# kakaobrain/rq-vae-transformer

Hardware: AMD Instinct MI355X
Metric: 256x256 images/sec, AR sampling + decode (RQ-Transformer huge, 8x8x4 codes) (higher is better)
Workload: dtype bf16

## Files before the change

rq-vae-transformer_amd/csrc/conv_halo.hip:

```cpp
#include <stdlib.h>
#include <type_traits>
#include "gemm.h"
#include "rq_common.h"
#include "vae_kernels.h"
#ifndef RQ_CONV_NT
#define RQ_CONV_NT 0
#endif
#ifndef RQ_CONVOUT_NT
#define RQ_CONVOUT_NT 0
#endif
static __device__ __forceinline__ rq_u128 ld128_act(const void* p) {
#if RQ_CONV_NT >= 2
    return ld128_nt(p);
#else
    return ld128(p);
#endif
}
static __device__ __forceinline__ void st128_act(void* p, rq_u128 v) {
#if RQ_CONV_NT >= 1
    st128_nt(p, v);
#else
    st128(p, v);
#endif
}

struct ConvHaloArgs {
    const bf16_t* x;
    const bf16_t* w;
    const float* bias;
    const float* gn;
    const bf16_t* resid;
    bf16_t* out;
    float* stats;
    int B, H, W, Cin, Cout;
};

#define RQ_LOG2E 1.4426950408889634f
static __device__ __forceinline__ float rq_silu_l2(float t) { return t * rq_fast_rcp(fmaf(rq_fast_exp2(-t), RQ_LOG2E, RQ_LOG2E)); }

static __device__ __forceinline__ void rq_stats_piece(const rq_u128& u, float (&sum)[4], float (&sq)[4]) {
    const uint32_t w[4] = {u.x, u.y, u.z, u.w};
#pragma unroll
    for (int e = 0; e < 4; ++e) {
        sum[e] = rq_dot2_bf16(w[e], RQ_ONE_X2, sum[e]);
        sq[e] = rq_dot2_bf16(w[e], w[e], sq[e]);
    }
}

constexpr int HT_H = 8, HT_W = 32;
constexpr int HP_W = HT_W + 2;
constexpr int H_BN = 128;
constexpr int HW_BYTES = H_BN * 128;
#ifndef RQ_HALO_WDMA
#define RQ_HALO_WDMA 1
#endif
#ifndef RQ_HALO_PMID
#define RQ_HALO_PMID 0
#endif
#ifndef RQ_HALO_RMID
#define RQ_HALO_RMID 1
#endif
#ifndef RQ_HALO_RES_F32
#define RQ_HALO_RES_F32 1
#endif
constexpr int H_WSLOTS = RQ_HALO_WDMA ? 4 : 3;
constexpr int H_SMEM_BYTES = 2 * (HT_H + 2) * HP_W * 128 + H_WSLOTS * HW_BYTES;
static __device__ __forceinline__ void halo_wait_dma(int nd, int no) {
#define RQ_HC(ND, K) case K: rq_wait_vmcnt_mixed<ND, K>(); break;
#define RQ_HW(ND) switch (no) { RQ_HC(ND, 0) RQ_HC(ND, 1) RQ_HC(ND, 2) RQ_HC(ND, 3) RQ_HC(ND, 4) RQ_HC(ND, 5) RQ_HC(ND, 6) RQ_HC(ND, 7) RQ_HC(ND, 8) \
    RQ_HC(ND, 9) RQ_HC(ND, 10) RQ_HC(ND, 11) RQ_HC(ND, 12) default: rq_wait_vmcnt_mixed<ND, 0>(); break; }
    if (nd >= 2) { RQ_HW(2) } else { RQ_HW(0) }
#undef RQ_HW
#undef RQ_HC
}

template <int PW = HP_W>
static __device__ __forceinline__ unsigned halo_lds_off(int hy, int hx, int c8) {
    return (unsigned)((hy * PW + hx) * 128 + ((c8 ^ ((hx >> 1) & 7)) << 4));
}

#ifdef RQ_CONV_TRACE
__device__ unsigned long long g_conv_trace[8 * 64];
#define RQ_CT(slot) do { if (blockIdx.x == RQ_CONV_TRACE && lane == 0 && (slot) < 64) g_conv_trace[wave * 64 + (slot)] = __builtin_readcyclecounter(); } while (0)
#else
#define RQ_CT(slot) do { } while (0)
#endif
template <int FUSE_GN, int UPS, int RES>
__global__ __launch_bounds__(512, 1) void conv3x3_halo_kernel(ConvHaloArgs p) {
    constexpr bool WDMA = RQ_HALO_WDMA != 0;
    constexpr int TH = HT_H, NTH = 512, RPW = 2, NJ = 2, W_IT = 2, TPX = TH * HT_W, W_SETS = 3, W_SLOTS = H_WSLOTS;
    static_assert(!(FUSE_GN && UPS), "the upsample conv has no Normalize in front of it");
    constexpr int PW = UPS ? HT_W / 2 + 2 : HP_W, PH = UPS ? TH / 2 + 2 : TH + 2;
    constexpr int HP_N = PW * PH;
    constexpr int HALO_BYTES = HP_N * 128;
    constexpr int H_IT = (HP_N * 8 + NTH - 1) / NTH;
    RQ_DYN_SMEM(smem);
    char* sH = (char*)smem;
    char* sW = sH + 2 * HALO_BYTES;
    const int tid = threadIdx.x, lane = tid & 63, wave = tid >> 6;
    const int wm = wave >> 1, wn = wave & 1;
#ifdef RQ_CONV_TRACE
    if (blockIdx.x == RQ_CONV_TRACE && lane == 0) g_conv_trace[wave * 64 + 58] = __builtin_amdgcn_s_memrealtime();
#endif

    const int tiles_x = p.W / HT_W, tiles_y = p.H / TH, NT = p.Cout / H_BN;
    const int n_mt = p.B * tiles_y * tiles_x;
    const int id = blockIdx.x, xcd = id & 7, slot = id >> 3;
    const int per = (n_mt + 7) >> 3;
    const int mtile = xcd * per + slot / NT;
    const int nt = slot - (slot / NT) * NT;
    if (slot >= per * NT || mtile >= n_mt) return;
    const int img = mtile / (tiles_y * tiles_x);
    const int trem = mtile - img * (tiles_y * tiles_x);
    const int ty0 = (trem / tiles_x) * TH, tx0 = (trem - (trem / tiles_x) * tiles_x) * HT_W;
    const int n0 = nt * H_BN;

    const char* gX = (const char*)p.x;
    const char* gWt = (const char*)p.w;
    const int w_row = tid >> 3, w_c8 = tid & 7;
    unsigned w_goff[W_IT];
#pragma unroll
    for (int i = 0; i < W_IT; ++i) w_goff[i] = (unsigned)(((long)(n0 + w_row + (NTH / 8) * i) * 9 * p.Cin + w_c8 * 8) * 2);
    auto load_w = [&](int c, int tap, rq_u128* rw) {
        const unsigned kb = (unsigned)(tap * p.Cin + c * 64) * 2u;
#pragma unroll
        for (int i = 0; i < W_IT; ++i) rw[i] = ld128(gWt + (w_goff[i] + kb));
    };
    rq_u128 rh[H_IT], rw[W_SETS][W_IT], r01[2][W_IT];
    unsigned w_voff[2];
#pragma unroll
    for (int i = 0; i < 2; ++i) {
        const int r = wave * 16 + i * 8 + (lane >> 3);
        w_voff[i] = (unsigned)(((long)(n0 + r) * 9 * p.Cin + ((lane & 7) ^ ((r >> 1) & 7)) * 8) * 2);
    }
    const rq_lds_t sW_dma = rq_lds_addr(sW) + (rq_lds_t)rq_uniform(wave) * 2048u;
    auto dma_w = [&](int c, int tap, unsigned woff) {
        if (tap >= 9) { tap -= 9; ++c; }
        rq_glds16_s2(sW_dma + woff, gWt + (unsigned)rq_uniform((tap * p.Cin + c * 64) * 2), w_voff[0], w_voff[1]);
    };
    if (WDMA) {
        dma_w(0, 0, 0u);
        dma_w(0, 1, (unsigned)HW_BYTES);
        dma_w(0, 2, 2u * HW_BYTES);
    } else {
        load_w(0, 0, r01[0]);
        load_w(0, 1, r01[1]);
        load_w(0, 2, rw[2]);
        load_w(0, 3, rw[0]);
        load_w(0, 4, rw[1]);
    }
    rq_sched_barrier();

    unsigned hd[H_IT];
    const int Hs = UPS ? p.H >> 1 : p.H, Ws = UPS ? p.W >> 1 : p.W;
    const unsigned x_img = (unsigned)((long)img * Hs * Ws * p.Cin * 2) + (unsigned)((tid & 7) * 16);
    const unsigned cin2 = (unsigned)p.Cin * 2u;
    const int hp0 = tid >> 3, hy0 = hp0 / PW, hx0 = hp0 - hy0 * PW;
    {
        int hy = hy0, hx = hx0;
#pragma unroll
        for (int it = 0; it < H_IT; ++it) {
            const int gy = (UPS ? ty0 >> 1 : ty0) + hy - 1, gx = (UPS ? tx0 >> 1 : tx0) + hx - 1;
            const int cy = gy < 0 ? 0 : (gy >= Hs ? Hs - 1 : gy), cx = gx < 0 ? 0 : (gx >= Ws ? Ws - 1 : gx);
            hd[it] = (unsigned)(cy * Ws + cx);
            rh[it] = ld128_act(gX + (x_img + hd[it] * cin2));
            hy += (NTH / 8) / PW; hx += (NTH / 8) % PW;
            if (hx >= PW) { hx -= PW; ++hy; }
        }
    }
    const float* gn = FUSE_GN ? p.gn + (long)img * p.Cin * 2 : nullptr;
    f32x4 gs[4];
    auto load_gs = [&](int c) {
        if (FUSE_GN) {
#pragma unroll
            for (int e = 0; e < 4; ++e) gs[e] = *(const f32x4*)(gn + (c * 64 + (tid & 7) * 8 + e * 2) * 2);
        }
    };
    auto scale_gs = [&]() {
        if (FUSE_GN) {
#pragma unroll
            for (int e = 0; e < 4; ++e) { rq_opaque_f4(gs[e]); gs[e] = gs[e] * RQ_LOG2E; }
        }
    };
    load_gs(0);
    rq_sched_barrier();
    {
        int hp = hp0, hy = hy0, hx = hx0;
        const int c8 = tid & 7;
#pragma unroll
        for (int it = 0; it < H_IT; ++it) {
            const bool in = hp < HP_N;
            const int gy = (UPS ? ty0 >> 1 : ty0) + hy - 1, gx = (UPS ? tx0 >> 1 : tx0) + hx - 1;
            const bool ok = in && gy >= 0 && gy < Hs && gx >= 0 && gx < Ws;
            const unsigned loff16 = in ? halo_lds_off<PW>(hy, hx, c8) >> 4 : 0u;
            hd[it] |= (loff16 << 16) | (ok ? 1u << 29 : 0u) | (in ? 1u << 30 : 0u);
            hp += NTH / 8; hy += (NTH / 8) / PW; hx += (NTH / 8) % PW;
            if (hx >= PW) { hx -= PW; ++hy; }
        }
    }
    auto h_in = [&](int it) { return (hd[it] >> 30) & 1u; };
    auto h_ok = [&](int it) { return (hd[it] >> 29) & 1u; };
    auto h_loff = [&](int it) { return ((hd[it] >> 16) & 0x1fffu) << 4; };
    auto h_goff = [&](int it) { return x_img + (hd[it] & 0xffffu) * cin2; };
    auto load_halo_piece = [&](int c, rq_u128* rh, int it) { rh[it] = ld128_act(gX + (h_goff(it) + (unsigned)c * 128u)); };

    unsigned w_loff[W_IT];
#pragma unroll
    for (int i = 0; i < W_IT; ++i) {
        const int r = w_row + (NTH / 8) * i;
        w_loff[i] = (unsigned)(r * 128 + ((w_c8 ^ ((r >> 1) & 7)) << 4));
    }
    auto halo_piece_value = [&](const rq_u128* rh, int it) -> rq_u128 {
        rq_u128 v = rh[it];
        if (FUSE_GN) {
            float f[8];
            rq_unpack2(v.x, f[0], f[1]);
            rq_unpack2(v.y, f[2], f[3]);
            rq_unpack2(v.z, f[4], f[5]);
            rq_unpack2(v.w, f[6], f[7]);
#pragma unroll
            for (int e = 0; e < 8; e += 2) {
                const f32x4 ss = gs[e >> 1];
                const float a = fmaf(f[e], ss[0], ss[1]), b = fmaf(f[e + 1], ss[2], ss[3]);
                f[e] = rq_silu_l2(a);
                f[e + 1] = rq_silu_l2(b);
            }
            v.x = pack_bf16x2(f[0], f[1]); v.y = pack_bf16x2(f[2], f[3]);
            v.z = pack_bf16x2(f[4], f[5]); v.w = pack_bf16x2(f[6], f[7]);
        }
        if (!h_ok(it)) v = zero128();
        return v;
    };
    auto halo_word = [&](rq_u128* rh, int it, int e) -> uint32_t& { return e == 0 ? rh[it].x : e == 1 ? rh[it].y : e == 2 ? rh[it].z : rh[it].w; };
    auto halo_piece_word = [&](rq_u128* rh, int it, int e) {
        uint32_t& w = halo_word(rh, it, e);
        if (FUSE_GN) {
            const f32x4 ss = gs[e];
            float wlo, whi;
            rq_unpack2(w, wlo, whi);
            const float a = fmaf(wlo, ss[0], ss[1]), b = fmaf(whi, ss[2], ss[3]);
            w = pack_bf16x2(rq_silu_l2(a), rq_silu_l2(b));
        }
        if (!h_ok(it)) w = 0u;
    };
    auto store_w = [&](int wslot, const rq_u128* rw) {
#pragma unroll
        for (int i = 0; i < W_IT; ++i) st128(sW + wslot * HW_BYTES + w_loff[i], rw[i]);
    };

    f32x16 acc[RPW][NJ];
#pragma unroll
    for (int j = 0; j < NJ; ++j)
#pragma unroll
        for (int q = 0; q < 4; ++q) {
            const f32x4 bv = *(const f32x4*)(p.bias + n0 + wn * (NJ * 32) + j * 32 + 8 * q + 4 * (lane >> 5));
#pragma unroll
            for (int i = 0; i < RPW; ++i)
#pragma unroll
                for (int e = 0; e < 4; ++e) acc[i][j][4 * q + e] = bv[e];
        }

    const int ftx = lane & 31, fk = lane >> 5;
    const unsigned rd_w0 = (unsigned)((wn * (NJ * 32) + ftx) * 128 + ((fk ^ ((ftx >> 1) & 7)) << 4));
    unsigned rd_h0[3];
#pragma unroll
    for (int kx = 0; kx < 3; ++kx)
        rd_h0[kx] = UPS ? halo_lds_off<PW>(wm * (RPW / 2), (ftx + kx + 1) >> 1, fk) : halo_lds_off<PW>(wm * RPW, ftx + kx, fk);

    auto load_frags = [&](int hbuf, unsigned woff, int ky, int kx, int ks, bf16x8* af, bf16x8* bfr) {
        const char* hb = sH + ((rd_h0[kx] + (unsigned)(hbuf * HALO_BYTES)) ^ (unsigned)(ks << 5));
        const char* wb = sW + ((rd_w0 ^ (unsigned)(ks << 5)) + woff);
#pragma unroll
        for (int i = 0; i < RPW; ++i) af[i] = as_bf16x8(ld128(hb + (UPS ? (i + ky + 1) >> 1 : i + ky) * (PW * 128)));
#pragma unroll
        for (int j = 0; j < NJ; ++j) bfr[j] = as_bf16x8(ld128(wb + j * (32 * 128)));
    };
#ifndef RQ_HALO_FDEPTH
#define RQ_HALO_FDEPTH 1
#endif
    constexpr int FD = RQ_HALO_FDEPTH, NSET = FD + 1;
    static_assert(FD >= 1 && FD <= 3 && 36 % NSET == 0, "fragment read-ahead of 1..3 k-steps");
    bf16x8 fa[NSET][RPW], fb[NSET][NJ];
    auto mfma_step = [&](int set) {
#pragma unroll
        for (int i = 0; i < RPW; ++i)
#pragma unroll
            for (int j = 0; j < NJ; ++j) acc[i][j] = rq_mfma_32x32x16_bf16(fb[set][j], fa[set][i], acc[i][j]);
    };

    const int NC = p.Cin / 64, last_c = NC - 1;
    auto load_unit = [&](int c, int tap, rq_u128* r) {
        if (tap >= 9) { tap -= 9; ++c; }
        if (c > last_c) return false;
        load_w(c, tap, r);
        return true;
    };
    {
        RQ_CT(0);
        scale_gs();
#pragma unroll
        for (int it = 0; it < H_IT; ++it)
            if (h_in(it)) st128(sH + h_loff(it), halo_piece_value(rh, it));
        if (WDMA) rq_wait_vmcnt_mixed<0, 0>();
// ... 537 lines not shown
                for (int k = 0; k < PPT; ++k) {
                    const int it = (tap - FIRST) * PPT + k;
                    if (ptap && it < H_IT) rh[it] = halo_piece_value(rh, it);
                }
                compute(hbuf, wbuf, ky, kx, rh, -1);
            }
            store_w(wbuf ^ 1, rw[(tap + 1) % W_SETS]);
#pragma unroll
            for (int k = 0; k < PPT; ++k) {
                const int it = (tap - FIRST) * PPT + k;
                if (!(ptap && it < H_IT)) continue;
                if (h_in(it)) st128(sH + (hbuf ^ 1) * PK_PSTRIDE + h_loff(it), rh[it]);
            }
            RQ_CTP(2 + (c * 9 + tap) * 2);
            rq_syncthreads();
            RQ_CTP(3 + (c * 9 + tap) * 2);
            wbuf ^= 1;
        }
        hbuf ^= 1;
    };

    for (;;) {
        rq_opaque(tid_o);
        static_assert(CPR == 16 && NTH / CPR == HT_W && R_IT == TH, "piece k = tile row k");
        if (SUB)
            io_off0 = (unsigned)((((long)cur.img * p.H + 2 * cur.ty0 + (cur.cls >> 1)) * p.W + 2 * (cur.tx0 + (tid_o >> 4)) + (cur.cls & 1)) * p.Cout + cur.n0 + (tid_o & 15) * 8) * 2u;
        else
            io_off0 = (unsigned)((((long)cur.img * p.H + cur.ty0) * p.W + cur.tx0 + (tid_o >> 4)) * p.Cout + cur.n0 + (tid_o & 15) * 8) * 2u;
        RQ_CTP(1);
        for (int c = 0; c + 1 < NC; ++c) run_chunk(c, std::false_type{});
        run_chunk(NC - 1, std::true_type{});

        char* sT = (char*)smem + PK_P0 + (hbuf == 0 ? PK_PATCH : 0);
        const int lane_o = tid_o & 63, wave_o = tid_o >> 6, wm_o = wave_o >> 1, wn_o = wave_o & 1;
        float* sred = (float*)(sT + PK_TILE);
        if (RES) {
#pragma unroll
            for (int k = 0; k < R_IT; ++k) st128(sT + ((tid_o >> 4) + HT_W * k) * PK_LDR + (tid_o & 15) * 16, rr[k]);
            rq_syncthreads();
        }
#pragma unroll
        for (int i = 0; i < RPW; ++i) {
            const int ty = wm_o * RPW + i, tx = lane_o & 31;
            const int ml = ty * HT_W + tx;
#pragma unroll
            for (int j = 0; j < 2; ++j) {
#pragma unroll
                for (int q = 0; q < 4; ++q) {
                    const int nl = wn_o * 64 + j * 32 + 8 * q + 4 * (lane_o >> 5);
                    float v[4];
#pragma unroll
                    for (int e = 0; e < 4; ++e) v[e] = acc[i][j][4 * q + e];
                    if (RES) {
                        const uint32_t* rp = (const uint32_t*)(sT + ml * PK_LDR + nl * 2);
                        const uint32_t r0 = rp[0], r1 = rp[1];
                        { float lo_, hi_; rq_unpack2(r0, lo_, hi_); v[0] += lo_; v[1] += hi_; }
                        { float lo_, hi_; rq_unpack2(r1, lo_, hi_); v[2] += lo_; v[3] += hi_; }
                    }
                    struct __attribute__((aligned(8))) u64 { uint32_t a, b; } w2;
                    w2.a = pack_bf16x2(v[0], v[1]);
                    w2.b = pack_bf16x2(v[2], v[3]);
                    *(u64*)(sT + ml * PK_LDR + nl * 2) = w2;
                }
            }
        }
        if (has_next) acc_from_bias(nxt.n0);
        rq_syncthreads();
        RQ_CTP(61);
        float gs_[4], gq_[4];
#pragma unroll
        for (int e = 0; e < 4; ++e) { gs_[e] = 0.f; gq_[e] = 0.f; }
#pragma unroll
        for (int k = 0; k < R_IT; ++k) {
            const rq_u128 u = ld128(sT + ((tid_o >> 4) + HT_W * k) * PK_LDR + (tid_o & 15) * 16);
            st128_act((char*)p.out + (io_off0 + (unsigned)k * io_step), u);
            if (p.stats) rq_stats_piece(u, gs_, gq_);
        }
        if (p.stats) {
            const int gsz = p.Cout / 32;
            float a0, q0, a1, q1;
            if (gsz == 4) {
                a0 = gs_[0] + gs_[1]; q0 = gq_[0] + gq_[1];
                a1 = gs_[2] + gs_[3]; q1 = gq_[2] + gq_[3];
            } else {
                a0 = (gs_[0] + gs_[1]) + (gs_[2] + gs_[3]);
                q0 = (gq_[0] + gq_[1]) + (gq_[2] + gq_[3]);
                a1 = 0.f; q1 = 0.f;
            }
            a0 += rq_shfl_xor(a0, 16); q0 += rq_shfl_xor(q0, 16); a1 += rq_shfl_xor(a1, 16); q1 += rq_shfl_xor(q1, 16);
            a0 += rq_shfl_xor(a0, 32); q0 += rq_shfl_xor(q0, 32); a1 += rq_shfl_xor(a1, 32); q1 += rq_shfl_xor(q1, 32);
            if (lane_o < 16) {
                float* o = sred + (wave_o * 16 + lane_o) * 4;
                o[0] = a0; o[1] = q0; o[2] = a1; o[3] = q1;
            }
            rq_syncthreads();
            if (wave_o == 0) {
                const int chunk = (lane_o >> 1) & 15, pair = lane_o & 1;
                float a = 0.f, q = 0.f;
#pragma unroll
                for (int w = 0; w < NTH / 64; ++w) { a += sred[(w * 16 + chunk) * 4 + pair * 2]; q += sred[(w * 16 + chunk) * 4 + pair * 2 + 1]; }
                if (gsz == 16) {
                    a += rq_shfl_xor(a, 2);
                    q += rq_shfl_xor(q, 2);
                }
                const bool writer = gsz == 4 ? true : (gsz == 8 ? pair == 0 : (pair == 0 && (chunk & 1) == 0));
                if (writer && lane_o < 32) {
                    const int g = (cur.n0 + chunk * 8 + pair * 4) / gsz;
                    const int tiles = tiles_x * tiles_y * NCLS;
                    float* o = p.stats + (((long)cur.img * tiles + cur.trem) * 32 + g) * 2;
                    o[0] = a;
                    o[1] = q;
                }
            }
        }
        RQ_CTP(63);
#ifdef RQ_CONV_TRACE
        ++trace_tile;
#endif
        if (!has_next) break;
        rq_use(rw[1][0].x, rw[1][1].x, rw[2][0].x, rw[2][1].x);
        if (SUB) rq_use(rw[W_SETS - 1][0].x, rw[W_SETS - 1][1].x, rw[W_SETS - 1][0].y, rw[W_SETS - 1][1].y);
        rq_use(acc[0][0][0], acc[RPW - 1][1][15]);
        slot += wpx;
        cur = nxt;
        wn_cur = wn_nxt;
        if (SUB) set_class(cur.cls);
        has_next = slot_ok(slot + wpx);
        if (has_next) { nxt = decode(slot + wpx); wn_nxt = (unsigned)nxt.n0 * w_per_n + (unsigned)nxt.cls * w_per_cls; }
    }
}

struct ConvOutArgs {
    const bf16_t* x;
    const float* w;
    const float* bias;
    const float* gn;
    float* y;
    int B, H, W, Cin, Cout;
};
constexpr int OT_H = 4, OP_N = (OT_H + 2) * HP_W;
constexpr int O_NTH = 256;
constexpr int O_PLANE = OP_N * 128;

template <int FUSE_GN>
__global__ __launch_bounds__(O_NTH) void conv_out_halo_kernel(ConvOutArgs p) {
    RQ_DYN_SMEM(smem);
    const int NC = p.Cin / 64;
    char* sH = (char*)smem;
    const int wrow = 9 * p.Cin * 2 + 32;
    char* sW = sH + NC * O_PLANE;
    const int tid = threadIdx.x, lane = tid & 63, wave = rq_uniform(tid >> 6);

    const int tiles_x = p.W / HT_W, tiles_y = p.H / OT_H, tiles_img = tiles_x * tiles_y;
    const int n_mt = p.B * tiles_img;
    const int id = blockIdx.x, xcd = id & 7, slot = id >> 3, S = (int)gridDim.x >> 3;
    const int per = (n_mt + 7) >> 3;
    const int x0 = xcd * per, x1 = x0 + per < n_mt ? x0 + per : n_mt;
    const int sub = (x1 - x0 + S - 1) / (S > 0 ? S : 1);
    const int t0 = x0 + slot * sub, t1 = t0 + sub < x1 ? t0 + sub : x1;
    if (x0 >= x1 || t0 >= t1) return;

    const int cpp_sh = p.Cin == 64 ? 3 : 4;
    const int CPP = 1 << cpp_sh;
    const int cq = tid & (CPP - 1);
    const int n_piece = OP_N << cpp_sh;
    constexpr int PIT = 13;
    unsigned hyx[PIT];
#pragma unroll
    for (int k = 0; k < PIT; ++k) {
        const int q = tid + O_NTH * k;
        const int hp = q >> cpp_sh;
        const int hy = hp / HP_W, hx = hp - hy * HP_W;
        hyx[k] = q < n_piece ? (unsigned)(hy << 8 | hx) : 0xffffu;
    }
    const char* gX = (const char*)p.x;
    struct Tile { int img, ty0, tx0; };
    auto decode = [&](int t) {
        Tile d;
        d.img = t / tiles_img;
        const int trem = t - d.img * tiles_img;
        d.ty0 = (trem / tiles_x) * OT_H;
        d.tx0 = (trem - (trem / tiles_x) * tiles_x) * HT_W;
        return d;
    };
    auto request = [&](const Tile& d, rq_u128* r, f32x4* gs) {
        if (FUSE_GN) {
            const float* gn = p.gn + ((long)d.img * p.Cin + cq * 8) * 2;
#pragma unroll
            for (int e = 0; e < 4; ++e) gs[e] = *(const f32x4*)(gn + e * 4) * RQ_LOG2E;
        }
#pragma unroll
        for (int k = 0; k < PIT; ++k) {
            if (hyx[k] == 0xffffu) continue;
            const int gy = d.ty0 + (int)(hyx[k] >> 8) - 1, gx = d.tx0 + (int)(hyx[k] & 255u) - 1;
            const int cy = gy < 0 ? 0 : (gy >= p.H ? p.H - 1 : gy), cx = gx < 0 ? 0 : (gx >= p.W ? p.W - 1 : gx);
#if RQ_CONVOUT_NT
            r[k] = ld128_nt(gX + ((((long)d.img * p.H + cy) * p.W + cx) * p.Cin + cq * 8) * 2);
#else
            r[k] = ld128(gX + ((((long)d.img * p.H + cy) * p.W + cx) * p.Cin + cq * 8) * 2);
#endif
        }
    };
    auto stage = [&](const Tile& d, const rq_u128* r, const f32x4* gs) {
#pragma unroll
        for (int k = 0; k < PIT; ++k) {
            if (hyx[k] == 0xffffu) continue;
            const int hy = (int)(hyx[k] >> 8), hx = (int)(hyx[k] & 255u);
            const int gy = d.ty0 + hy - 1, gx = d.tx0 + hx - 1;
            rq_u128 v = r[k];
            if (FUSE_GN) {
                float f[8];
                rq_unpack2(v.x, f[0], f[1]);
                rq_unpack2(v.y, f[2], f[3]);
                rq_unpack2(v.z, f[4], f[5]);
                rq_unpack2(v.w, f[6], f[7]);
#pragma unroll
                for (int e = 0; e < 8; e += 2) {
                    const f32x4 ss = gs[e >> 1];
                    const float a = fmaf(f[e], ss[0], ss[1]), b = fmaf(f[e + 1], ss[2], ss[3]);
                    f[e] = rq_silu_l2(a);
                    f[e + 1] = rq_silu_l2(b);
                }
                v.x = pack_bf16x2(f[0], f[1]); v.y = pack_bf16x2(f[2], f[3]);
                v.z = pack_bf16x2(f[4], f[5]); v.w = pack_bf16x2(f[6], f[7]);
            }
            if (gy < 0 || gy >= p.H || gx < 0 || gx >= p.W) v = zero128();
            st128(sH + (unsigned)((cq >> 3) * O_PLANE) + halo_lds_off(hy, hx, cq & 7), v);
        }
    };

    rq_u128 r[PIT];
    f32x4 gs[4];
    Tile cur = decode(t0);
    request(cur, r, gs);
    const int KT = 9 * p.Cin;
    const int n_w4 = p.Cout * (KT >> 2);
    constexpr int WIT = 5;
    {
        f32x4 wr[WIT];
#pragma unroll
        for (int k = 0; k < WIT; ++k) {
            const int i = tid + O_NTH * k;
            if (i < n_w4) wr[k] = *(const f32x4*)(p.w + (long)i * 4);
        }
        stage(cur, r, gs);
#pragma unroll
        for (int k = 0; k < WIT; ++k) {
            const int i = tid + O_NTH * k;
            if (i < n_w4) {
                const int row = i / (KT >> 2), k4 = (i - row * (KT >> 2)) * 4;
                *(uint64_t*)(sW + row * wrow + k4 * 2) = (uint64_t)pack_bf16x2(wr[k][0], wr[k][1]) | ((uint64_t)pack_bf16x2(wr[k][2], wr[k][3]) << 32);
            }
        }
        for (int i = n_w4 + tid; i < 8 * (KT >> 2); i += O_NTH) {
            const int row = i / (KT >> 2), k4 = (i - row * (KT >> 2)) * 4;
            *(uint64_t*)(sW + row * wrow + k4 * 2) = 0ull;
        }
    }

    const int ftx = lane & 31, fk = lane >> 5;
    const char* wl = sW + (ftx & 7) * wrow + fk * 16;
    float bias_r[4];
#pragma unroll
    for (int co = 0; co < 4; ++co) bias_r[co] = co < p.Cout ? p.bias[co] : 0.f;
    for (int t = t0; t < t1; ++t) {
        const bool more = t + 1 < t1;
        Tile nxt = cur;
        if (more) { nxt = decode(t + 1); request(nxt, r, gs); }
        rq_syncthreads();
        f32x16 acc;
#pragma unroll
        for (int q = 0; q < 16; ++q) acc[q] = 0.f;
        constexpr int OD = 4;
        for (int c = 0; c < NC; ++c) {
            bf16x8 af[OD + 1], wf[OD + 1];
            auto frag = [&](int s, bf16x8& a, bf16x8& w) {
                const int tap = s >> 2, ks = s & 3, ky = tap / 3, kx = tap - ky * 3;
                const unsigned ha = (unsigned)(c * O_PLANE) + halo_lds_off(wave + ky, ftx + kx, fk);
                a = as_bf16x8(ld128(sH + (ha ^ (unsigned)(ks << 5))));
                w = as_bf16x8(ld128(wl + (tap * p.Cin + c * 64) * 2 + ks * 32));
            };
#pragma unroll
            for (int s = 0; s < OD; ++s) frag(s, af[s], wf[s]);
#pragma unroll
            for (int s = 0; s < 36; ++s) {
                if (s + OD < 36) frag(s + OD, af[(s + OD) % (OD + 1)], wf[(s + OD) % (OD + 1)]);
                acc = rq_mfma_32x32x16_bf16(wf[s % (OD + 1)], af[s % (OD + 1)], acc);
                rq_sched_barrier();
            }
        }
        if (lane < 32) {
            const int oy = cur.ty0 + wave, ox = cur.tx0 + lane;
#pragma unroll
            for (int co = 0; co < 4; ++co)
                if (co < p.Cout) p.y[(((long)cur.img * p.Cout + co) * p.H + oy) * p.W + ox] = acc[co] + bias_r[co];
        }
        if (!more) break;
        rq_syncthreads();
        stage(nxt, r, gs);
        cur = nxt;
    }
}

bool rq_conv_out_halo_supported(int H, int W, int Cin, int Cout) {
    return H % OT_H == 0 && W % HT_W == 0 && (Cin == 64 || Cin == 128) && Cout >= 1 && Cout <= 4;
}

int rq_launch_conv_out_halo(const bf16_t* x, const float* w, const float* bias, const float* gn, float* y, int B, int H, int W,
                            int Cin, int Cout, hipStream_t s) {
    if (!rq_conv_out_halo_supported(H, W, Cin, Cout)) return rq_fail(RQAMD_ERR_UNSUPPORTED, "conv_out_halo: shape %dx%d %d->%d", H, W, Cin, Cout);
    ConvOutArgs a{};
    a.x = x; a.w = w; a.bias = bias; a.gn = gn; a.y = y; a.B = B; a.H = H; a.W = W; a.Cin = Cin; a.Cout = Cout;
    const size_t smem = (size_t)(Cin / 64) * O_PLANE + 8 * (size_t)(9 * Cin * 2 + 32);
    static RqDeviceOnce attr_once;
    if (attr_once.first()) {
        (void)hipFuncSetAttribute((const void*)conv_out_halo_kernel<0>, hipFuncAttributeMaxDynamicSharedMemorySize, 160 * 1024);
        (void)hipFuncSetAttribute((const void*)conv_out_halo_kernel<1>, hipFuncAttributeMaxDynamicSharedMemorySize, 160 * 1024);
    }
    const int n_mt = B * (H / OT_H) * (W / HT_W);
    int nblocks = 8 * ((n_mt + 7) / 8);
    int cus = 256;
    (void)hipDeviceGetAttribute(&cus, hipDeviceAttributeMultiprocessorCount, 0);
    if (nblocks > 2 * cus) nblocks = 2 * cus / 8 * 8;
    if (const char* e = getenv("RQAMD_CONV_OUT_WGS")) {
        const int v = atoi(e) / 8 * 8;
        if (v >= 8 && v < nblocks) nblocks = v;
    }
    if (gn) RQ_LAUNCH(conv_out_halo_kernel<1>, dim3(nblocks), dim3(O_NTH), smem, s, a);
    else RQ_LAUNCH(conv_out_halo_kernel<0>, dim3(nblocks), dim3(O_NTH), smem, s, a);
    return rq_check_launch("conv_out_halo_kernel");
}

struct ConvInArgs {
    const float* x;
    const float* w;
    const float* bias;
    bf16_t* y;
    float* stats;
    int B, H, W;
};
constexpr int CI_COUT = 128, CI_PATCH = 3 * (HT_H + 2) * HP_W;
constexpr int CI_WROW = 80;
constexpr int CI_STG = 32 * (CI_COUT * 2 + 16);

__global__ __launch_bounds__(256) void conv_in_mfma_kernel(ConvInArgs p) {
    RQ_DYN_SMEM(smem);
    float* sP = (float*)smem;
    int* sK = (int*)(smem + 4096);
    char* sWt = (char*)smem + 4096 + 128;
    char* sO = sWt + CI_COUT * CI_WROW;
    const int tid = threadIdx.x, lane = tid & 63, wave = rq_uniform(tid >> 6);
    const int tiles_x = p.W / HT_W, tiles_y = p.H / HT_H;
    const int tile = blockIdx.x;
    const int img = tile / (tiles_y * tiles_x), trem = tile - img * (tiles_y * tiles_x);
    const int ty0 = (trem / tiles_x) * HT_H, tx0 = (trem - (trem / tiles_x) * tiles_x) * HT_W;

    for (int i = tid; i < CI_PATCH + 4; i += 256) {
        float v = 0.f;
        if (i < CI_PATCH) {
            const int ci = i / ((HT_H + 2) * HP_W), r = i - ci * ((HT_H + 2) * HP_W);
            const int hy = r / HP_W, hx = r - hy * HP_W;
            const int gy = ty0 + hy - 1, gx = tx0 + hx - 1;
            if (gy >= 0 && gy < p.H && gx >= 0 && gx < p.W) v = p.x[(((long)img * 3 + ci) * p.H + gy) * p.W + gx];
        }
        sP[i] = v;
    }
    if (tid < 32) {
        const int k = tid, tap = k / 3, ci = k - tap * 3, ky = tap / 3, kx = tap - ky * 3;
        sK[k] = k < 27 ? ci * ((HT_H + 2) * HP_W) + ky * HP_W + kx : -1;
    }
    for (int i = tid; i < CI_COUT * 16; i += 256) {
        const int co = i >> 4, k2 = (i & 15) * 2;
        const float a = k2 < 27 ? p.w[k2 * CI_COUT + co] : 0.f, b = k2 + 1 < 27 ? p.w[(k2 + 1) * CI_COUT + co] : 0.f;
        *(uint32_t*)(sWt + co * CI_WROW + k2 * 2) = pack_bf16x2(a, b);
    }
    rq_syncthreads();

    const int px = lane & 31, g = lane >> 5;
    int koff[2][8];
#pragma unroll
    for (int ks = 0; ks < 2; ++ks)
#pragma unroll
        for (int e = 0; e < 8; ++e) koff[ks][e] = sK[ks * 16 + g * 8 + e];
    bf16x8 bfr[2][4];
#pragma unroll
    for (int ks = 0; ks < 2; ++ks)
#pragma unroll
        for (int j = 0; j < 4; ++j) bfr[ks][j] = as_bf16x8(ld128(sWt + (j * 32 + px) * CI_WROW + (ks * 16 + g * 8) * 2));
    char* stg = sO + wave * CI_STG;
    float gs_[4] = {0.f, 0.f, 0.f, 0.f}, gq_[4] = {0.f, 0.f, 0.f, 0.f};
#pragma unroll 1
    for (int i = 0; i < 2; ++i) {
        const int row = wave * 2 + i;
        f32x16 acc[4];
#pragma unroll
        for (int j = 0; j < 4; ++j)
#pragma unroll
            for (int r = 0; r < 16; ++r) acc[j][r] = 0.f;
#pragma unroll
        for (int ks = 0; ks < 2; ++ks) {
            float f[8];
#pragma unroll
            for (int e = 0; e < 8; ++e) f[e] = koff[ks][e] >= 0 ? sP[koff[ks][e] + row * HP_W + px] : 0.f;
            rq_u128 u;
            u.x = pack_bf16x2(f[0], f[1]); u.y = pack_bf16x2(f[2], f[3]);
            u.z = pack_bf16x2(f[4], f[5]); u.w = pack_bf16x2(f[6], f[7]);
            const bf16x8 af = as_bf16x8(u);
#pragma unroll
            for (int j = 0; j < 4; ++j) acc[j] = rq_mfma_32x32x16_bf16(bfr[ks][j], af, acc[j]);
        }
#pragma unroll
        for (int j = 0; j < 4; ++j)
#pragma unroll
            for (int q = 0; q < 4; ++q) {
                const int co = j * 32 + 8 * q + 4 * g;
                const f32x4 bv = *(const f32x4*)(p.bias + co);
                struct __attribute__((aligned(8))) u64 { uint32_t a, b; } w2;
                w2.a = pack_bf16x2(acc[j][4 * q] + bv[0], acc[j][4 * q + 1] + bv[1]);
                w2.b = pack_bf16x2(acc[j][4 * q + 2] + bv[2], acc[j][4 * q + 3] + bv[3]);
                *(u64*)(stg + px * (CI_COUT * 2 + 16) + co * 2) = w2;
            }
        rq_syncthreads();
        const long pix0 = ((long)img * p.H + ty0 + row) * p.W + tx0;
#pragma unroll
        for (int k = 0; k < 8; ++k) {
            const int c = lane + 64 * k, opx = c >> 4, part = c & 15;
            const rq_u128 u = ld128(stg + opx * (CI_COUT * 2 + 16) + part * 16);
            st128(p.y + (pix0 + opx) * CI_COUT + part * 8, u);
            if (p.stats) rq_stats_piece(u, gs_, gq_);
        }
        rq_syncthreads();
    }
    if (p.stats) {
        float a0 = gs_[0] + gs_[1], q0 = gq_[0] + gq_[1], a1 = gs_[2] + gs_[3], q1 = gq_[2] + gq_[3];
        a0 += rq_shfl_xor(a0, 16); q0 += rq_shfl_xor(q0, 16); a1 += rq_shfl_xor(a1, 16); q1 += rq_shfl_xor(q1, 16);
        a0 += rq_shfl_xor(a0, 32); q0 += rq_shfl_xor(q0, 32); a1 += rq_shfl_xor(a1, 32); q1 += rq_shfl_xor(q1, 32);
        float* sred = (float*)sO;
        if (lane < 16) {
            float* o = sred + (wave * 16 + lane) * 4;
            o[0] = a0; o[1] = q0; o[2] = a1; o[3] = q1;
        }
        rq_syncthreads();
        if (tid < 32) {
            const int chunk = tid >> 1, pair = tid & 1;
            float a = 0.f, q = 0.f;
#pragma unroll
            for (int w = 0; w < 4; ++w) { a += sred[(w * 16 + chunk) * 4 + pair * 2]; q += sred[(w * 16 + chunk) * 4 + pair * 2 + 1]; }
            float* o = p.stats + (((long)img * (tiles_y * tiles_x) + trem) * 32 + tid) * 2;
            o[0] = a;
            o[1] = q;
        }
    }
}

bool rq_conv_in_mfma_supported(int H, int W, int Cin, int Cout) {
    return Cin == 3 && Cout == CI_COUT && H % HT_H == 0 && W % HT_W == 0;
}

int rq_launch_conv_in_mfma(const float* x, const float* w, const float* bias, bf16_t* y, float* stats, int B, int H, int W, hipStream_t s) {
    ConvInArgs a{};
    a.x = x; a.w = w; a.bias = bias; a.y = y; a.stats = stats; a.B = B; a.H = H; a.W = W;
    const size_t smem = 4096 + 128 + (size_t)CI_COUT * CI_WROW + 4 * (size_t)CI_STG;
    static RqDeviceOnce attr_once;
    if (attr_once.first()) {
        (void)hipFuncSetAttribute((const void*)conv_in_mfma_kernel, hipFuncAttributeMaxDynamicSharedMemorySize, (int)smem);
    }
    RQ_LAUNCH(conv_in_mfma_kernel, dim3((unsigned)(B * (H / HT_H) * (W / HT_W))), dim3(256), smem, s, a);
    return rq_check_launch("conv_in_mfma_kernel");
}

__global__ __launch_bounds__(256) void gn_params_kernel(const float* part, const float* gamma, const float* beta, float* gn, int B, int HW,
                                                        int C, int nchunk, float eps) {
    __shared__ float sa[8][32], sq[8][32], smean[32], srstd[32];
    const int b = blockIdx.x, tid = threadIdx.x, g = tid & 31, sl = tid >> 5;
    float a = 0.f, q = 0.f;
    for (int c = sl; c < nchunk; c += 8) {
        const float* o = part + (((long)b * nchunk + c) * 32 + g) * 2;
        a += o[0];
        q += o[1];
    }
    sa[sl][g] = a;
    sq[sl][g] = q;
    rq_syncthreads();
    if (tid < 32) {
        float ta = 0.f, tq = 0.f;
#pragma unroll
        for (int k = 0; k < 8; ++k) { ta += sa[k][tid]; tq += sq[k][tid]; }
        const float n = (float)HW * (float)(C / 32);
        const float mean = ta / n;
        float var = tq / n - mean * mean;
        if (var < 0.f) var = 0.f;
        smean[tid] = mean;
        srstd[tid] = 1.0f / sqrtf(var + eps);
    }
    rq_syncthreads();
    const int cpg = C / 32;
    for (int ch = tid; ch < C; ch += 256) {
        const int gg = ch / cpg;
        const float sc = srstd[gg] * gamma[ch];
        gn[((long)b * C + ch) * 2] = sc;
        gn[((long)b * C + ch) * 2 + 1] = beta[ch] - smean[gg] * sc;
    }
}

__global__ void ups_subpixel_weights_kernel(const bf16_t* w, bf16_t* wsub, int Cout, int Cin) {
    const long n = (long)4 * Cout * 4 * Cin;
    const long gid = (long)blockIdx.x * blockDim.x + threadIdx.x;
    if (gid >= n) return;
    const int ci = (int)(gid % Cin);
    long r = gid / Cin;
    const int tap = (int)(r & 3); r >>= 2;
    const int co = (int)(r % Cout);
    const int cls = (int)(r / Cout);
    const int py = cls >> 1, px = cls & 1, a = tap >> 1, b = tap & 1;
    const int ky_lo = py == 0 ? (a == 0 ? 0 : 1) : (a == 0 ? 0 : 2), ky_hi = py == 0 ? (a == 0 ? 0 : 2) : (a == 0 ? 1 : 2);
    const int kx_lo = px == 0 ? (b == 0 ? 0 : 1) : (b == 0 ? 0 : 2), kx_hi = px == 0 ? (b == 0 ? 0 : 2) : (b == 0 ? 1 : 2);
    float acc = 0.f;
    for (int ky = ky_lo; ky <= ky_hi; ++ky)
        for (int kx = kx_lo; kx <= kx_hi; ++kx) acc += bf16_to_f32(w[(((long)co * 3 + ky) * 3 + kx) * Cin + ci]);
    wsub[gid] = f32_to_bf16(acc);
}
int rq_launch_ups_subpixel_weights(const bf16_t* w, bf16_t* wsub, int Cout, int Cin, hipStream_t s) {
    const long n = (long)16 * Cout * Cin;
    RQ_LAUNCH(ups_subpixel_weights_kernel, dim3((unsigned)((n + 255) / 256)), dim3(256), 0, s, w, wsub, Cout, Cin);
    return rq_check_launch("ups_subpixel_weights_kernel");
}
bool rq_conv_halo_subpixel_supported(int H, int W, int Cin, int Cout) {
    return rq_conv_halo_supported(H, W, Cin, Cout) && (H >> 1) % HT_H == 0 && (W >> 1) % HT_W == 0;
}

bool rq_conv_halo_supported(int H, int W, int Cin, int Cout) {
    return H % HT_H == 0 && W % HT_W == 0 && Cin % 64 == 0 && Cout % H_BN == 0 && H >= 32 && H * W <= 65536;
}

int rq_conv_halo_stat_tiles(int H, int W) { return (H / HT_H) * (W / HT_W); }
static int g_conv_halo_dbg_pk = 0;
static int g_conv_halo_dbg_wpx = 0;
static bool halo_persistent(int ups) {
    static const int env = getenv("RQAMD_HALO_PERSIST") ? atoi(getenv("RQAMD_HALO_PERSIST")) : -1;
    if (g_conv_halo_dbg_pk) return g_conv_halo_dbg_pk > 0;
    return env < 0 ? ups != 0 : env != 0;
}

static int launch_conv_halo_th(const ConvHaloArgs& a, int ups, hipStream_t s) {
    constexpr int TH = HT_H, NTHR = 512;
    constexpr size_t smem = H_SMEM_BYTES;
    static_assert((size_t)TH * HT_W * (H_BN * 2 + 16) + 4096 <= H_SMEM_BYTES, "the epilogue tile overlays the operand buffers");
    static RqDeviceOnce attr_once;
    if (attr_once.first()) {
        (void)hipFuncSetAttribute((const void*)conv3x3_halo_kernel<0, 0, 0>, hipFuncAttributeMaxDynamicSharedMemorySize, (int)smem);
        (void)hipFuncSetAttribute((const void*)conv3x3_halo_kernel<0, 0, 1>, hipFuncAttributeMaxDynamicSharedMemorySize, (int)smem);
        (void)hipFuncSetAttribute((const void*)conv3x3_halo_kernel<1, 0, 0>, hipFuncAttributeMaxDynamicSharedMemorySize, (int)smem);
        (void)hipFuncSetAttribute((const void*)conv3x3_halo_kernel<1, 0, 1>, hipFuncAttributeMaxDynamicSharedMemorySize, (int)smem);
        (void)hipFuncSetAttribute((const void*)conv3x3_halo_kernel<0, 1, 0>, hipFuncAttributeMaxDynamicSharedMemorySize, (int)smem);
    }
    const int n_mt = a.B * (a.H / TH) * (a.W / HT_W), NT = a.Cout / H_BN;
    const int nblocks = 8 * ((n_mt + 7) / 8) * NT;
    if (ups == 2) {
        static RqDeviceOnce sub_once;
        static int cus_per_xcd_s[16];
        int dev = 0;
        (void)hipGetDevice(&dev);
        if (sub_once.first()) {
            (void)hipFuncSetAttribute((const void*)conv3x3_halo_pk_kernel<0, 2, 0>, hipFuncAttributeMaxDynamicSharedMemorySize, PK_SMEM);
            int cus = 0;
            if (hipDeviceGetAttribute(&cus, hipDeviceAttributeMultiprocessorCount, dev) != hipSuccess || cus < 8) cus = 256;
            cus_per_xcd_s[dev & 15] = cus / 8;
        }
        const int n_sub = a.B * ((a.H >> 1) / TH) * ((a.W >> 1) / HT_W) * 4;
        const int slots = ((n_sub + 7) / 8) * NT;
        int wpx = g_conv_halo_dbg_wpx > 0 ? g_conv_halo_dbg_wpx : cus_per_xcd_s[dev & 15];
        if (wpx > slots) wpx = slots;
        RQ_LAUNCH((conv3x3_halo_pk_kernel<0, 2, 0>), dim3(8 * wpx), dim3(512), PK_SMEM, s, a, wpx);
        return rq_check_launch("conv3x3_halo_pk_kernel<subpixel>");
    }
    if (ups && halo_persistent(ups)) {
        static RqDeviceOnce pk_once;
        static int cus_per_xcd[16];
        int dev = 0;
        (void)hipGetDevice(&dev);
        if (pk_once.first()) {
            (void)hipFuncSetAttribute((const void*)conv3x3_halo_pk_kernel<0, 1, 0>, hipFuncAttributeMaxDynamicSharedMemorySize, PK_SMEM);
            int cus = 0;
            if (hipDeviceGetAttribute(&cus, hipDeviceAttributeMultiprocessorCount, dev) != hipSuccess || cus < 8) cus = 256;
            cus_per_xcd[dev & 15] = cus / 8;
        }
        const int slots = ((n_mt + 7) / 8) * NT;
        int wpx = g_conv_halo_dbg_wpx > 0 ? g_conv_halo_dbg_wpx : cus_per_xcd[dev & 15];
        if (wpx > slots) wpx = slots;
        RQ_LAUNCH((conv3x3_halo_pk_kernel<0, 1, 0>), dim3(8 * wpx), dim3(512), PK_SMEM, s, a, wpx);
        return rq_check_launch("conv3x3_halo_pk_kernel");
    }
    if (ups) RQ_LAUNCH((conv3x3_halo_kernel<0, 1, 0>), dim3(nblocks), dim3(NTHR), smem, s, a);
    else if (a.gn && a.resid) RQ_LAUNCH((conv3x3_halo_kernel<1, 0, 1>), dim3(nblocks), dim3(NTHR), smem, s, a);
    else if (a.gn) RQ_LAUNCH((conv3x3_halo_kernel<1, 0, 0>), dim3(nblocks), dim3(NTHR), smem, s, a);
    else if (a.resid) RQ_LAUNCH((conv3x3_halo_kernel<0, 0, 1>), dim3(nblocks), dim3(NTHR), smem, s, a);
    else RQ_LAUNCH((conv3x3_halo_kernel<0, 0, 0>), dim3(nblocks), dim3(NTHR), smem, s, a);
    return rq_check_launch("conv3x3_halo_kernel");
}

int rq_launch_conv_halo(const bf16_t* x, const bf16_t* w, const float* bias, const float* gn, const bf16_t* resid, bf16_t* out,
                        float* stats, int B, int H, int W, int Cin, int Cout, int ups, hipStream_t s) {
    if (stats && Cout != 128 && Cout != 256 && Cout != 512) return rq_fail(RQAMD_ERR_UNSUPPORTED, "conv_halo: fused statistics need Cout 128/256/512");
    if (!rq_conv_halo_supported(H, W, Cin, Cout)) return rq_fail(RQAMD_ERR_UNSUPPORTED, "conv_halo: shape %dx%d %d->%d", H, W, Cin, Cout);
    if (ups && (gn || resid)) return rq_fail(RQAMD_ERR_UNSUPPORTED, "conv_halo: the upsample conv takes no GroupNorm / residual");
    if (ups == 2 && !rq_conv_halo_subpixel_supported(H, W, Cin, Cout)) return rq_fail(RQAMD_ERR_UNSUPPORTED, "conv_halo: sub-pixel form at %dx%d", H, W);
    if (2.0 * B * H * W * (Cin > Cout ? Cin : Cout) >= 4294967296.0) return rq_fail(RQAMD_ERR_UNSUPPORTED, "conv_halo: tensor larger than 4 GiB");
    ConvHaloArgs a{};
    a.x = x; a.w = w; a.bias = bias; a.gn = gn; a.resid = resid; a.out = out; a.stats = stats; a.B = B; a.H = H; a.W = W; a.Cin = Cin; a.Cout = Cout;
    return launch_conv_halo_th(a, ups, s);
}

int rq_launch_gn_params(const bf16_t* x, float* part, const float* gamma, const float* beta, float* gn, int B, int HW, int C,
                        int nchunk_have, hipStream_t s) {
    int nchunk = nchunk_have;
// ... 41 lines not shown
```

Before: 1594.

## Add per-tap GEMM conv_out kernel with shared-memory tap reduction as default

Adds a new conv_out kernel that, for each input pixel, computes all 9*Cout tap products with one MFMA per K-slice, then sums the shifted tap contributions from a rolling shared-memory row buffer to form the 3x3 output. Halo edge columns are handled as separate items. The kernel also overlaps the next pixel's global loads with the current compute, splits work into column strips with row segments spread across XCDs, and fuses the GroupNorm+SiLU prologue. It becomes the default path unless RQAMD_CONV_OUT=halo is set. In exchange it adds extra shared-memory traffic and block-wide syncs per output row, and the large shared buffer limits occupancy.

Result: no change. 1606 (median of 6 runs) (+0.7%).

```diff
diff --git a/rq-vae-transformer_amd/csrc/conv_halo.hip b/rq-vae-transformer_amd/csrc/conv_halo.hip
--- a/rq-vae-transformer_amd/csrc/conv_halo.hip
+++ b/rq-vae-transformer_amd/csrc/conv_halo.hip
@@ -1,4 +1,5 @@
 #include <stdlib.h>
+#include <string.h>
 #include <type_traits>
 #include "gemm.h"
 #include "rq_common.h"
@@ -1142,6 +1143,195 @@
     }
 }
 
+constexpr int TP_NTH = 256, TP_SEG = 8;
+constexpr int TP_EROWS = OT_H * TP_SEG + 2;
+#ifndef RQ_TAPS_OCC
+#define RQ_TAPS_OCC 3
+#endif
+constexpr int TP_OCC = RQ_TAPS_OCC;
+
+template <int FUSE_GN, int NB, int KS>
+__global__ __launch_bounds__(TP_NTH, NB == 1 ? TP_OCC : 2) void conv_out_taps_kernel(ConvOutArgs p, int seg) {
+    RQ_DYN_SMEM(smem);
+    constexpr int CIN = 16 * KS, chalf = CIN / 2;
+    constexpr int PS = 32 * NB + 1;
+    float* sG = (float*)smem;
+    float* sP = sG + 256;
+    float* sE = sP + 6 * 32 * PS;
+    const int tid = threadIdx.x, lane = tid & 63, wave = rq_uniform(tid >> 6);
+    const int px = lane & 31, hf = lane >> 5;
+    const int ncol = 9 * p.Cout;
+
+    const int tiles_x = p.W / HT_W, tiles_y = p.H / OT_H, nseg = (tiles_y + seg - 1) / seg, units_img = nseg * tiles_x;
+    const int n_u = p.B * units_img;
+    const int id = blockIdx.x, xcd = id & 7, slot = id >> 3, S = (int)gridDim.x >> 3;
+    const int per = (n_u + 7) >> 3;
+    const int x0 = xcd * per, x1 = x0 + per < n_u ? x0 + per : n_u;
+    const int sub = (x1 - x0 + S - 1) / (S > 0 ? S : 1);
+    const int u0 = x0 + slot * sub, u1 = u0 + sub < x1 ? u0 + sub : x1;
+    if (x0 >= x1 || u0 >= u1) return;
+
+    const char* gX = (const char*)p.x;
+    struct Unit { int img, gy0, tx0, n; };
+    auto decode = [&](int u) {
+        Unit d;
+        d.img = u / units_img;
+        const int rem = u - d.img * units_img, sg = rem / tiles_x;
+        d.gy0 = sg * seg * OT_H;
+        d.tx0 = (rem - sg * tiles_x) * HT_W;
+        d.n = tiles_y - sg * seg < seg ? tiles_y - sg * seg : seg;
+        return d;
+    };
+    auto n_edge = [&](const Unit& U) { return (2 * (OT_H * U.n + 2) + 31) >> 5; };
+    auto n_first = [&](const Unit& U) { return (n_edge(U) + 6 - wave + 3) >> 2; };
+    auto item = [&](const Unit& U, int pos, int& edge, int& idx) {
+        const int nE = n_edge(U), cntP = n_first(U);
+        if (pos < cntP) { const int i = wave + 4 * pos; edge = i < nE; idx = edge ? i : i - nE; }
+        else { edge = 0; idx = OT_H * (pos - cntP + 1) + 2 + wave; }
+    };
+    auto pixel = [&](const Unit& U, int edge, int idx, int& g, int& gx, bool& has) {
+        if (!edge) { g = idx; gx = U.tx0 + px; has = true; }
+        else { const int q = 32 * idx + px; g = q >> 1; gx = (q & 1) ? U.tx0 + HT_W : U.tx0 - 1; has = g < OT_H * U.n + 2; }
+    };
+    auto request = [&](const Unit& U, int edge, int idx, rq_u128* r) {
+        int g, gx;
+        bool has;
+        pixel(U, edge, idx, g, gx, has);
+        const int gy = U.gy0 + g - 1;
+        const int cy = gy < 0 ? 0 : (gy >= p.H ? p.H - 1 : gy), cx = gx < 0 ? 0 : (gx >= p.W ? p.W - 1 : gx);
+        const char* src = gX + ((((long)U.img * p.H + cy) * p.W + cx) * CIN + hf * chalf) * 2;
+#pragma unroll
+        for (int ks = 0; ks < KS; ++ks) r[ks] = ld128(src + ks * 16);
+    };
+    auto load_gn = [&](int img) {
+        return tid < 2 * CIN ? p.gn[(long)img * CIN * 2 + tid] * RQ_LOG2E : 0.f;
+    };
+    const int g_slot = (tid >> 2) * 4 + (tid & 1) * 2 + ((tid >> 1) & 1);
+
+    rq_u128 ra[KS], rb[KS];
+#pragma unroll
+    for (int ks = 0; ks < KS; ++ks) rb[ks] = zero128();
+    Unit cur = decode(u0);
+    {
+        int e, i;
+        item(cur, 0, e, i);
+        request(cur, e, i, ra);
+    }
+    if (FUSE_GN) sG[g_slot] = load_gn(cur.img);
+    bf16x8 wf[NB][KS];
+#pragma unroll
+    for (int nb = 0; nb < NB; ++nb) {
+        const int n = nb * 32 + px;
+        const int tap = n / p.Cout, co = n - tap * p.Cout;
+        const float* ws = p.w + ((long)(co * 9 + tap) * CIN + hf * chalf);
+#pragma unroll
+        for (int ks = 0; ks < KS; ++ks) {
+            rq_u128 u = zero128();
+            if (n < ncol) {
+                const f32x4 a = *(const f32x4*)(ws + ks * 8), c = *(const f32x4*)(ws + ks * 8 + 4);
+                u.x = pack_bf16x2(a[0], a[1]); u.y = pack_bf16x2(a[2], a[3]);
+                u.z = pack_bf16x2(c[0], c[1]); u.w = pack_bf16x2(c[2], c[3]);
+            }
+            wf[nb][ks] = as_bf16x8(u);
+        }
+    }
+    const int sy = (tid >> 5) & 3, sx = tid & 31;
+    float bias_r[2];
+#pragma unroll
+    for (int i = 0; i < 2; ++i) bias_r[i] = (tid >> 7) + 2 * i < p.Cout ? p.bias[(tid >> 7) + 2 * i] : 0.f;
+
+    auto block = [&](const Unit& U, int edge, int idx, const rq_u128* r) {
+        int g, gx;
+        bool has;
+        pixel(U, edge, idx, g, gx, has);
+        const int gy = U.gy0 + g - 1;
+        const bool inside = has && gy >= 0 && gy < p.H && gx >= 0 && gx < p.W;
+        f32x16 acc[NB];
+#pragma unroll
+        for (int nb = 0; nb < NB; ++nb)
+#pragma unroll
+            for (int q = 0; q < 16; ++q) acc[nb][q] = 0.f;
+#pragma unroll
+        for (int ks = 0; ks < KS; ++ks) {
+            rq_u128 v = r[ks];
+            if (FUSE_GN) {
+                const float* gt = sG + (hf * chalf + ks * 8) * 2;
+                float f[8];
+                rq_unpack2(v.x, f[0], f[1]);
+                rq_unpack2(v.y, f[2], f[3]);
+                rq_unpack2(v.z, f[4], f[5]);
+                rq_unpack2(v.w, f[6], f[7]);
+#pragma unroll
+                for (int e = 0; e < 8; e += 2) {
+                    const f32x4 ss = *(const f32x4*)(gt + e * 2);
+                    const float a = fmaf(f[e], ss[0], ss[2]), c = fmaf(f[e + 1], ss[1], ss[3]);
+                    f[e] = rq_silu_l2(a);
+                    f[e + 1] = rq_silu_l2(c);
+                }
+                v.x = pack_bf16x2(f[0], f[1]); v.y = pack_bf16x2(f[2], f[3]);
+                v.z = pack_bf16x2(f[4], f[5]); v.w = pack_bf16x2(f[6], f[7]);
+            }
+            if (!inside) v = zero128();
+#pragma unroll
+            for (int nb = 0; nb < NB; ++nb) acc[nb] = rq_mfma_32x32x16_bf16(wf[nb][ks], as_bf16x8(v), acc[nb]);
+        }
+        if (has) {
+            float* o = (edge ? sE + (g * 2 + (px & 1)) * PS : sP + ((idx % 6) * 32 + px) * PS) + 4 * hf;
+#pragma unroll
+            for (int nb = 0; nb < NB; ++nb)
+#pragma unroll
+                for (int q = 0; q < 16; ++q) o[nb * 32 + (q & 3) + 8 * (q >> 2)] = acc[nb][q];
+        }
+    };
+
+    for (int u = u0; u < u1; ++u) {
+        const bool more = u + 1 < u1;
+        Unit nxt = cur;
+        if (more) nxt = decode(u + 1);
+        float g_next = 0.f;
+        if (FUSE_GN && more) g_next = load_gn(nxt.img);
+        const int cntP = n_first(cur), cnt = cntP + cur.n - 1;
+        auto step = [&](int pos) {
+            int e, i, e2, i2;
+            item(cur, pos, e, i);
+            if (pos + 1 < cnt) { item(cur, pos + 1, e2, i2); request(cur, e2, i2, rb); }
+            else if (more) { item(nxt, 0, e2, i2); request(nxt, e2, i2, rb); }
+            block(cur, e, i, ra);
+#pragma unroll
+            for (int ks = 0; ks < KS; ++ks) ra[ks] = rb[ks];
+        };
+        rq_syncthreads();
+        for (int pos = 0; pos < cntP; ++pos) step(pos);
+        for (int k = 0; k < cur.n; ++k) {
+            if (k) {
+                rq_syncthreads();
+                step(cntP + k - 1);
+            }
+            rq_syncthreads();
+            const int g0 = OT_H * k + sy, s0 = g0 % 6;
+#pragma unroll
+            for (int i = 0; i < 2; ++i) {
+                const int co = (tid >> 7) + 2 * i;
+                if (co < p.Cout) {
+                    float v = bias_r[i];
+#pragma unroll
+                    for (int tap = 0; tap < 9; ++tap) {
+                        const int ky = tap / 3, hx = sx + tap % 3;
+                        const int sl = s0 + ky < 6 ? s0 + ky : s0 + ky - 6;
+                        const float* src = hx == 0 ? sE + ((g0 + ky) * 2) * PS
+                                                   : (hx == HP_W - 1 ? sE + ((g0 + ky) * 2 + 1) * PS : sP + (sl * 32 + hx - 1) * PS);
+                        v += src[tap * p.Cout + co];
+                    }
+                    p.y[(((long)cur.img * p.Cout + co) * p.H + cur.gy0 + g0) * p.W + cur.tx0 + sx] = v;
+                }
+            }
+        }
+        if (FUSE_GN && more) sG[g_slot] = g_next;
+        cur = nxt;
+    }
+}
+
+
 bool rq_conv_out_halo_supported(int H, int W, int Cin, int Cout) {
     return H % OT_H == 0 && W % HT_W == 0 && (Cin == 64 || Cin == 128) && Cout >= 1 && Cout <= 4;
 }
@@ -1151,6 +1341,43 @@
     if (!rq_conv_out_halo_supported(H, W, Cin, Cout)) return rq_fail(RQAMD_ERR_UNSUPPORTED, "conv_out_halo: shape %dx%d %d->%d", H, W, Cin, Cout);
     ConvOutArgs a{};
     a.x = x; a.w = w; a.bias = bias; a.gn = gn; a.y = y; a.B = B; a.H = H; a.W = W; a.Cin = Cin; a.Cout = Cout;
+    const char* sel = getenv("RQAMD_CONV_OUT");
+    if (!(sel && strcmp(sel, "halo") == 0)) {
+        const int nbk = 9 * Cout > 32 ? 2 : 1;
+        const size_t smem_t = (256 + (size_t)(6 * 32 + TP_EROWS * 2) * (32 * nbk + 1)) * sizeof(float);
+        static RqDeviceOnce taps_once;
+        if (taps_once.first()) {
+            (void)hipFuncSetAttribute((const void*)conv_out_taps_kernel<0, 2, 8>, hipFuncAttributeMaxDynamicSharedMemorySize, 160 * 1024);
+            (void)hipFuncSetAttribute((const void*)conv_out_taps_kernel<1, 2, 8>, hipFuncAttributeMaxDynamicSharedMemorySize, 160 * 1024);
+            (void)hipFuncSetAttribute((const void*)conv_out_taps_kernel<0, 2, 4>, hipFuncAttributeMaxDynamicSharedMemorySize, 160 * 1024);
+            (void)hipFuncSetAttribute((const void*)conv_out_taps_kernel<1, 2, 4>, hipFuncAttributeMaxDynamicSharedMemorySize, 160 * 1024);
+        }
+        int cus = 256;
+        (void)hipDeviceGetAttribute(&cus, hipDeviceAttributeMultiprocessorCount, 0);
+        const int occ = nbk == 1 ? TP_OCC : 2;
+        const int tiles_y = H / OT_H, strips = B * (W / HT_W);
+        int seg = TP_SEG;
+        while (seg > 1 && strips * ((tiles_y + seg - 1) / seg) < 2 * occ * cus) seg >>= 1;
+        if (const char* e = getenv("RQAMD_CONV_OUT_SEG")) {
+            const int v = atoi(e);
+            if (v >= 1 && v <= TP_SEG) seg = v;
+        }
+        const int n_u = strips * ((tiles_y + seg - 1) / seg);
+        int nblocks = 8 * ((n_u + 7) / 8);
+        if (nblocks > occ * cus) nblocks = occ * cus / 8 * 8;
+        if (const char* e = getenv("RQAMD_CONV_OUT_WGS")) {
+            const int v = atoi(e) / 8 * 8;
+            if (v >= 8 && v < nblocks) nblocks = v;
+        }
+#define RQ_TAPS(G, N) do { if (Cin == 128) RQ_LAUNCH((conv_out_taps_kernel<G, N, 8>), dim3(nblocks), dim3(TP_NTH), smem_t, s, a, seg); \
+                           else RQ_LAUNCH((conv_out_taps_kernel<G, N, 4>), dim3(nblocks), dim3(TP_NTH), smem_t, s, a, seg); } while (0)
+        if (gn && nbk == 1) RQ_TAPS(1, 1);
+        else if (gn) RQ_TAPS(1, 2);
+        else if (nbk == 1) RQ_TAPS(0, 1);
+        else RQ_TAPS(0, 2);
+#undef RQ_TAPS
+        return rq_check_launch("conv_out_taps_kernel");
+    }
     const size_t smem = (size_t)(Cin / 64) * O_PLANE + 8 * (size_t)(9 * Cin * 2 + 32);
     static RqDeviceOnce attr_once;
     if (attr_once.first()) {
```
